# etri/bwa-mem-scale

Hardware: AMD Instinct MI355X
Metric: Mreads/sec through the GPU hot path (seed -> chain -> extend -> dedup, reads and index resident), 150bp SE vs a synthetic genome of GRCh38 size, at 1 MI355X; % HBM roofline in roofline.frac (higher is better)
Workload: dtype int64 intervals / int16 DP (two columns per register; int32 for queries beyond 191 bases or scores beyond 2^14)

## Files before the change

bwa-mem-scale_amd/csrc/api_extend.hip:

```cpp
#include <cstddef>

#include "stage_state.h"

using namespace bwams;

extern "C" {
static int ext_args(bwams_batch *b, StageState *s, const bwams_mem_opt_t *opt, ExtArgs *A) {
    const int64_t n1 = s->ch.nseq + 1;
    A->chains = s->ch.chains.p; A->n_chains = s->ch.n_chains; A->seeds = s->ch.seeds.p; A->n_seeds = s->ch.n_seeds;
    A->chain_off = s->ch.chain_off.as<int64_t>(); A->seed_off = s->ch.chain_off.as<int64_t>() + n1; A->enc = b->d_enc.p; A->cum = b->d_cum.p;
    A->nseq = s->ch.nseq; A->ref = b->idx->fmi.ref;
    int rc = dev_bns(b->idx, &A->bns);
    if (rc) return rc;
    A->opt = *opt; A->regs = s->ext.regs.p; A->srt = s->ext.srt.p; A->rmax = s->ext.rmax.as<int64_t>(); A->cnt = s->ext.cnt.as<int32_t>();
    A->ctr = b->d_ctr.p; A->state = s->ext.state.p; A->kreg = s->ext.kreg.p; A->cur = s->ext.cur.p; A->lim = s->ext.lim.p; A->sel_heavy = s->heavy.p;
    A->n_sel_heavy = &b->d_ctr.p->sel_heavy; A->sel_ticket = b->d_ctr.p->ext_sel_ticket; A->req_list = s->ext.req_list.p; A->rtask = nullptr;
    return BWAMS_OK;
}

static hipError_t ext_round_clear(bwams_batch *b) {
    DevCounters *c = b->d_ctr.p;
    return hipMemsetAsync(&c->ext_n_req, 0, (size_t)((char *)(c->ext_n_retry + 2) - (char *)&c->ext_n_req), b->stream);
}
static int ext_round_fetch(bwams_batch *b, int64_t *n_req, int64_t *n_rest, int64_t *n_l, int64_t *n_r) {
    DevCounters *h = b->h_ctr.p;
    BWAMS_HIP(hipMemcpyAsync(&h->ext_n_req, &b->d_ctr.p->ext_n_req, 3 * sizeof(unsigned long long), hipMemcpyDeviceToHost, b->stream));
    BWAMS_HIP(hipStreamSynchronize(b->stream));
    *n_req = (int64_t)h->ext_n_req; *n_rest = (int64_t)h->ext_n_rest;
    *n_l = (int64_t)(h->ext_n_tasks & 0xffffffffull); *n_r = (int64_t)(h->ext_n_tasks >> 32);
    return BWAMS_OK;
}

static int ext_plan(bwams_batch *b, StageState *s, const bwams_mem_opt_t *opt, int extend_all, ExtArgs *A) {
    const int64_t N1 = s->ch.n_seeds + 1, n1 = s->ch.nseq + 1;
    BWAMS_HIP(s->ext.regs.ensure_n((size_t)N1)); BWAMS_HIP(s->ext.srt.ensure_n((size_t)N1));
    BWAMS_HIP(s->ext.rmax.ensure((size_t)(s->ch.n_chains + 1) * 16)); BWAMS_HIP(s->ext.cnt.ensure((size_t)N1 * 6 * 4));
    BWAMS_HIP(s->ext.state.ensure_n((size_t)N1)); BWAMS_HIP(s->ext.kreg.ensure((size_t)N1 * 32)); BWAMS_HIP(s->ext.cur.ensure_n((size_t)n1));
    BWAMS_HIP(s->ext.lim.ensure_n((size_t)n1)); BWAMS_HIP(s->heavy.ensure_n((size_t)n1));
    BWAMS_HIP(s->ext.req_list.ensure_n((size_t)N1)); BWAMS_HIP(s->ext.rtask.ensure_n((size_t)N1));
    int rc = ext_args(b, s, opt, A);
    if (rc) return rc;
    BWAMS_HIP(hipMemsetAsync(&b->d_ctr.p->sel_heavy, 0, sizeof(unsigned long long), b->stream));
    BWAMS_HIP(ext_round_clear(b));
    launch_ext_heavy_list(*A, b->stream);
    BWAMS_HIP(hipMemsetAsync(s->ext.cur.p, 0, (size_t)n1 * 4, b->stream));
    BWAMS_HIP(hipMemsetAsync(s->ext.lim.p, 0, (size_t)n1 * 4, b->stream));
    launch_ext_plan(*A, extend_all, b->stream);
    return BWAMS_OK;
}

static int ext_build_flat(bwams_batch *b, StageState *s, const ExtArgs &A, const int32_t *list, int64_t n, int64_t tot[6]) {
    hipStream_t st = b->stream;
    const int64_t n1 = n + 1;
    BWAMS_HIP(s->ext.ewide.ensure((size_t)n1 * 6 * 8)); BWAMS_HIP(s->ext.eoffs.ensure((size_t)n1 * 6 * 8));
    launch_ext_widen(A, list, n, s->ext.ewide.as<int64_t>(), st);
    int rc = scan_rows(b, s->ext.ewide.as<int64_t>(), s->ext.eoffs.as<int64_t>(), 6, n1);
    if (rc) return rc;
    for (int r = 0; r < 6; ++r) BWAMS_HIP(hipMemcpyAsync(&tot[r], s->ext.eoffs.as<int64_t>() + r * n1 + n, 8, hipMemcpyDeviceToHost, st));
    BWAMS_HIP(hipStreamSynchronize(st));
    for (int r : {1, 2, 4, 5})
        if (tot[r] >= ((int64_t)1 << 31)) {
            set_last_error("extension task buffers exceed the 31-bit offsets of SeqPair; use smaller chunks");
            return BWAMS_ERR_CAPACITY;
        }
    s->ext.n_left = tot[0]; s->ext.lqer_b = tot[1]; s->ext.lref_b = tot[2];
    s->ext.n_right = tot[3]; s->ext.rqer_b = tot[4]; s->ext.rref_b = tot[5];
    BWAMS_HIP(s->ext.lpairs.ensure_n((size_t)(tot[0] + 1))); BWAMS_HIP(s->ext.rpairs.ensure_n((size_t)(tot[3] + 1)));
    const int64_t mx = tot[0] > tot[3] ? tot[0] : tot[3];
    BWAMS_HIP(s->ext.retry.ensure_n((size_t)(mx + 1)));
    s->ext.tasks_inplace = false;
    BWAMS_HIP(s->ext.lqer.ensure_n((size_t)tot[1] + 64)); BWAMS_HIP(s->ext.lref.ensure_n((size_t)tot[2] + 64));
    BWAMS_HIP(s->ext.rqer.ensure_n((size_t)tot[4] + 64)); BWAMS_HIP(s->ext.rref.ensure_n((size_t)tot[5] + 64));
    if (tot[0] + tot[3] > 0)
        launch_ext_build(A, list, n, s->ext.eoffs.as<int64_t>(), s->ext.lpairs.p, s->ext.lref.p, s->ext.lqer.p, s->ext.rpairs.p, s->ext.rref.p,
                         s->ext.rqer.p, nullptr, nullptr, st);
    return BWAMS_OK;
}

static int ext_build_round(bwams_batch *b, StageState *s, const ExtArgs &A, int64_t n_req, int64_t n_l, int64_t n_r, bool inplace) {
    if (!inplace) {
        int64_t tot[6] = {0, 0, 0, 0, 0, 0};
        if (int rc = ext_build_flat(b, s, A, A.req_list, n_req, tot)) return rc;
        if (tot[0] != n_l || tot[3] != n_r) {
            set_last_error("bwams_extend_run: the request list and its task counters disagree");
            return BWAMS_ERR_DEVICE;
        }
        return BWAMS_OK;
    }
    s->ext.n_left = n_l; s->ext.n_right = n_r;
    s->ext.lqer_b = s->ext.lref_b = s->ext.rqer_b = s->ext.rref_b = 0;
    BWAMS_HIP(s->ext.lpairs.ensure_n((size_t)(n_l + 1))); BWAMS_HIP(s->ext.rpairs.ensure_n((size_t)(n_r + 1)));
    const int64_t mx = n_l > n_r ? n_l : n_r;
    BWAMS_HIP(s->ext.retry.ensure_n((size_t)(mx + 1)));
    s->ext.tasks_inplace = true;
    BWAMS_HIP(s->ext.lsrc.ensure((size_t)(n_l + 1) * 16)); BWAMS_HIP(s->ext.rsrc.ensure((size_t)(n_r + 1) * 16));
    if (n_l + n_r > 0) launch_ext_build(A, A.req_list, n_req, nullptr, s->ext.lpairs.p, nullptr, nullptr, s->ext.rpairs.p,
                         nullptr, nullptr, s->ext.lsrc.as<int64_t>(), s->ext.rsrc.as<int64_t>(), b->stream);
    return BWAMS_OK;
}

int bwams_extend_build(bwams_batch_t *b, const bwams_mem_opt_t *opt, int64_t *n_left, int64_t *n_right) {
    if (!b || !b->stages || !b->stages->ch.done) {
        set_last_error("bwams_extend_build: run bwams_chain_run (or bwams_chain_upload) first");
        return BWAMS_ERR_ARG;
    }
    if (!b->idx->fmi.ref) {
        set_last_error("bwams_extend_build: the index was opened without its .0123 reference");
        return BWAMS_ERR_ARG;
    }
    int rc = check_opt(opt, "bwams_extend_build");
    if (rc) return rc;
    BWAMS_HIP(hipSetDevice(b->idx->device));
    StageState *s = b->stages;
    outdated(s, From::built);
    hipStream_t st = b->stream;
    ExtArgs A;
    BWAMS_HIP(hipEventRecord(s->ev[2], st));
    if ((rc = ext_plan(b, s, opt, 1, &A))) return rc;
    int64_t tot[6];
    if ((rc = ext_build_flat(b, s, A, nullptr, s->ch.n_seeds, tot))) return rc;
    BWAMS_HIP(hipEventRecord(s->ev[3], st));
    BWAMS_HIP(hipGetLastError());
    s->ext.built = true;
    s->opt = *opt;
    if (n_left) *n_left = tot[0];
    if (n_right) *n_right = tot[3];
    return BWAMS_OK;
}

static int run_side(bwams_batch *b, StageState *s, const ExtArgs &A, int right, int64_t *n_retry_out) {
    hipStream_t st = b->stream;
    bwams_seqpair_t *pairs = right ? s->ext.rpairs.p : s->ext.lpairs.p;
    const bool ip = s->ext.tasks_inplace;
    const uint8_t *ref = ip ? A.ref : (right ? s->ext.rref.p : s->ext.lref.p);
    const uint8_t *qer = ip ? A.enc : (right ? s->ext.rqer.p : s->ext.lqer.p);
    const int64_t *src = ip ? (right ? s->ext.rsrc.as<int64_t>() : s->ext.lsrc.as<int64_t>()) : nullptr;
    const int dir = ip && !right ? -1 : 1;
    const int64_t n = right ? s->ext.n_right : s->ext.n_left;
    SwParams prm;
    sw_params(A.opt, right ? A.opt.pen_clip3 : A.opt.pen_clip5, &prm);
    const int qmax = b->max_read_len > 1 ? b->max_read_len : 1;
    if (n == 0) return BWAMS_OK;
    unsigned long long *d_nretry = &b->d_ctr.p->ext_n_retry[right], *h_nretry = &b->h_ctr.p->ext_n_retry[right];
    bwams_seqpair_t *rp = A.rtask ? s->ext.rpairs.p : nullptr;
    if (bsw_list_bytes(n) > b->sw.d_bsw_list.cap) BWAMS_HIP(hipStreamSynchronize(st));
    BWAMS_HIP(b->sw.d_bsw_list.ensure(bsw_list_bytes(n), bsw_list_bytes(n + n / 4 + 1024)));
    if (int lrc = launch_bsw(pairs, n, ref, qer, A.opt.w, prm, qmax, b->d_ctr.p, b->cu_count, st, b->sw.d_bsw_list.p, s->aux, s->fork, s->join, src, dir)) {
        set_last_error(lrc == -2 ? "banded SW: a query longer than ~18000 bases does not fit the LDS kernel" : "banded SW: stream fork/join failed");
        return lrc == -2 ? BWAMS_ERR_UNSUPPORTED : BWAMS_ERR_DEVICE;
    }
    launch_ext_post(A, right, pairs, n, A.opt.w, 0, s->ext.retry.p, d_nretry, rp, st);
    BWAMS_HIP(hipMemcpyAsync(h_nretry, d_nretry, sizeof(unsigned long long), hipMemcpyDeviceToHost, st));
    BWAMS_HIP(hipStreamSynchronize(st));
    const unsigned long long nr = *h_nretry;
    if (nr) {
        if (launch_bsw(s->ext.retry.p, (int64_t)nr, ref, qer, A.opt.w << 1, prm, qmax, b->d_ctr.p, b->cu_count, st, b->sw.d_bsw_list.p, s->aux, s->fork, s->join, src, dir)) return BWAMS_ERR_DEVICE;
        launch_ext_post(A, right, s->ext.retry.p, (int64_t)nr, A.opt.w << 1, 1, nullptr, d_nretry, rp, st);
    }
    *n_retry_out += (int64_t)nr;
    return BWAMS_OK;
}

int bwams_extend_run(bwams_batch_t *b, const bwams_mem_opt_t *opt, int64_t *n_regs) {
    if (!b || !b->stages || !b->stages->ch.done) {
        set_last_error("bwams_extend_run: run bwams_chain_run (or bwams_chain_upload) first");
        return BWAMS_ERR_ARG;
    }
    if (!b->idx->fmi.ref) {
        set_last_error("bwams_extend_run: the index was opened without its .0123 reference");
        return BWAMS_ERR_ARG;
    }
    int rc = check_opt(opt, "bwams_extend_run");
    if (rc) return rc;
    int kMaxRounds = 6;
    if (knobs().ext_max_rounds > 0) kMaxRounds = knobs().ext_max_rounds;
    const bool adaptive_off = knobs().ext_all_rounds != 0;
    const bool inplace_on = knobs().ext_inplace != 0;
    StageState *s = b->stages;
    BWAMS_HIP(hipSetDevice(b->idx->device));
    hipStream_t st = b->stream;
    outdated(s, From::built);
    ExtArgs A;
    BWAMS_HIP(hipEventRecord(s->ev[10], st));
    BWAMS_HIP(hipMemsetAsync(&b->d_ctr.p->bsw_cells, 0, sizeof(unsigned long long), st));
    BWAMS_HIP(hipEventRecord(s->ev[2], st));
    if ((rc = ext_plan(b, s, opt, opt->extend_all != 0, &A))) return rc;
    A.rtask = s->ext.rtask.p;
    int64_t tot_left = 0, tot_right = 0;
    s->ext.n_retry_left = s->ext.n_retry_right = 0;
    int64_t n_req = 0, n_rest = 0, n_l = 0, n_r = 0;
    if ((rc = ext_round_fetch(b, &n_req, &n_rest, &n_l, &n_r))) return rc;
    int round = 0;
    for (;; ++round) {
        if ((rc = ext_build_round(b, s, A, n_req, n_l, n_r, inplace_on))) return rc;
        if (round == 0) { BWAMS_HIP(hipEventRecord(s->ev[3], st)); BWAMS_HIP(hipEventRecord(s->ev[4], st)); }
        tot_left += n_l; tot_right += n_r;
        if ((rc = run_side(b, s, A, 0, &s->ext.n_retry_left))) return rc;
        if (round == 0) { BWAMS_HIP(hipEventRecord(s->ev[5], st)); BWAMS_HIP(hipEventRecord(s->ev[6], st)); }
        if ((rc = run_side(b, s, A, 1, &s->ext.n_retry_right))) return rc;
        if (round == 0) { BWAMS_HIP(hipEventRecord(s->ev[7], st)); BWAMS_HIP(hipEventRecord(s->ev[8], st)); }
        BWAMS_HIP(ext_round_clear(b));
        const bool verbose_sel = knobs().verbose != 0;
        if (verbose_sel) BWAMS_HIP(hipMemsetAsync(b->d_ctr.p->dbg, 0, sizeof b->d_ctr.p->dbg, st));
        if (s->ch.n_seeds && launch_ext_select(A, b->cu_count, st, s->aux, s->fork, s->join)) {
            set_last_error("bwams_extend_run: stream fork/join failed");
            return BWAMS_ERR_DEVICE;
        }
        if (verbose_sel) {
            unsigned long long d[16];
            BWAMS_HIP(hipMemcpyAsync(d, b->d_ctr.p->dbg, sizeof d, hipMemcpyDeviceToHost, st));
            BWAMS_HIP(hipStreamSynchronize(st));
            if (d[0])
                fprintf(stderr, "[bwams_extend_run] selection walk, round %d: %llu reads, Mticks total %.2f fetch %.2f scan %.2f keep-anyway %.2f; %llu slots, %llu chunks, "
                                "%llu keep-anyway calls; longest read: %.3f Mticks (fetch %.3f scan %.3f keep %.3f), %llu slots %llu chunks %llu calls, %llu regions\n",
                        round, d[0], d[1] / 1e6, d[2] / 1e6, d[3] / 1e6, d[4] / 1e6, d[5], d[6], d[7], d[8] / 1e6, d[9] / 1e6, d[10] / 1e6, d[11] / 1e6, d[12], d[13], d[14], d[15]);
        }
        if (round == 0) BWAMS_HIP(hipEventRecord(s->ev[9], st));
        if ((rc = ext_round_fetch(b, &n_req, &n_rest, &n_l, &n_r))) return rc;
        if (n_req == 0) break;
        const bool few_left = !adaptive_off && (n_req + n_rest) * 32 < tot_left + tot_right;
        if (round + 1 >= kMaxRounds || few_left) {
            launch_ext_request_rest(A, st);
            if ((rc = ext_round_fetch(b, &n_req, &n_rest, &n_l, &n_r))) return rc;
        }
    }
    BWAMS_HIP(hipEventRecord(s->ev[11], st));
    BWAMS_HIP(hipGetLastError());
    s->ext.n_rounds = round + 1;
    s->ext.n_left = tot_left; s->ext.n_right = tot_right;
    s->ext.done = true;
    s->opt = *opt;
    if (n_regs) *n_regs = s->ch.n_seeds;
    return BWAMS_OK;
}

int bwams_extend_fetch(bwams_batch_t *b, bwams_alnreg_t *regs, int64_t reg_cap, int64_t *reg_off, int32_t *seed_aln) {
    if (!b || !b->stages || !(b->stages->ext.done || b->stages->ext.built)) {
        set_last_error("bwams_extend_fetch: no regions on the device");
        return BWAMS_ERR_ARG;
    }
    StageState *s = b->stages;
    if (s->ch.n_seeds > reg_cap) return BWAMS_ERR_CAPACITY;
    BWAMS_HIP(hipSetDevice(b->idx->device));
    hipStream_t st = b->stream;
    if (s->ch.n_seeds) BWAMS_HIP(hipMemcpyAsync(regs, s->ext.regs.p, (size_t)s->ch.n_seeds * sizeof(bwams_alnreg_t), hipMemcpyDeviceToHost, st));
    if (reg_off) BWAMS_HIP(hipMemcpyAsync(reg_off, s->ch.chain_off.as<int64_t>() + (s->ch.nseq + 1), (size_t)(s->ch.nseq + 1) * 8, hipMemcpyDeviceToHost, st));
    if (seed_aln && s->ch.n_seeds)
        BWAMS_HIP(hipMemcpy2DAsync(seed_aln, 4, reinterpret_cast<const char *>(s->ch.seeds.p) + offsetof(bwams_chain_seed_t, aln),
                                   sizeof(bwams_chain_seed_t), 4, (size_t)s->ch.n_seeds, hipMemcpyDeviceToHost, st));
    BWAMS_HIP(hipStreamSynchronize(st));
    return BWAMS_OK;
}

int bwams_extend_tasks_fetch(bwams_batch_t *b, int32_t side, bwams_seqpair_t *pairs, int64_t pair_cap, uint8_t *ref,
                             int64_t ref_cap, uint8_t *qer, int64_t qer_cap, int64_t *n_pairs, int64_t *ref_bytes,
                             int64_t *qer_bytes) {
    if (!b || !b->stages || !(b->stages->ext.built || b->stages->ext.done) || (side != 0 && side != 1)) {
        set_last_error("bwams_extend_tasks_fetch: no task lists on the device");
        return BWAMS_ERR_ARG;
    }
    if (b->stages->ext.tasks_inplace) {
        set_last_error("bwams_extend_tasks_fetch: bwams_extend_run extends in place and builds no flat task buffers; bwams_extend_build does");
        return BWAMS_ERR_ARG;
    }
    StageState *s = b->stages;
    const int64_t n = side ? s->ext.n_right : s->ext.n_left, rb = side ? s->ext.rref_b : s->ext.lref_b, qb = side ? s->ext.rqer_b : s->ext.lqer_b;
    if (n_pairs) *n_pairs = n;
    if (ref_bytes) *ref_bytes = rb;
    if (qer_bytes) *qer_bytes = qb;
    if (n > pair_cap || rb > ref_cap || qb > qer_cap) return BWAMS_ERR_CAPACITY;
    BWAMS_HIP(hipSetDevice(b->idx->device));
    hipStream_t st = b->stream;
    if (n) BWAMS_HIP(hipMemcpyAsync(pairs, side ? s->ext.rpairs.p : s->ext.lpairs.p, (size_t)n * sizeof(bwams_seqpair_t), hipMemcpyDeviceToHost, st));
    if (rb) BWAMS_HIP(hipMemcpyAsync(ref, side ? s->ext.rref.p : s->ext.lref.p, (size_t)rb, hipMemcpyDeviceToHost, st));
    if (qb) BWAMS_HIP(hipMemcpyAsync(qer, side ? s->ext.rqer.p : s->ext.lqer.p, (size_t)qb, hipMemcpyDeviceToHost, st));
    BWAMS_HIP(hipStreamSynchronize(st));
    return BWAMS_OK;
}
}
```

bwa-mem-scale_amd/csrc/ext_aln.hip:

```cpp
#include "common.h"
#include "chain_kernels.h"
#include "wave_ops.h"

namespace bwams {
namespace {

constexpr int H0_ = -99;
constexpr int kExtKept = 1, kExtPurged = 2, kExtReq = 4, kExtDone = 8;

__device__ __forceinline__ int cal_max_gap(const bwams_mem_opt_t &o, int qlen) {
    const int l_del = (int)((double)(qlen * o.a - o.o_del) / o.e_del + 1.);
    const int l_ins = (int)((double)(qlen * o.a - o.o_ins) / o.e_ins + 1.);
    int l = l_del > l_ins ? l_del : l_ins;
    l = l > 1 ? l : 1;
    return l < (o.w << 1) ? l : (o.w << 1);
}

__device__ __forceinline__ int pos2rid(const DevBns &b, int64_t pos_f) {
    int left = 0, mid = 0, right = b.n_seqs;
    if (pos_f >= b.l_pac) return -1;
    while (left < right) {
        mid = (left + right) >> 1;
        if (pos_f >= b.contigs[mid].offset) {
            if (mid == b.n_seqs - 1) break;
            if (pos_f < b.contigs[mid + 1].offset) break;
            left = mid + 1;
        } else right = mid;
    }
    return mid;
}

__device__ __forceinline__ int seedcov(const bwams_alnreg_t &a, const bwams_chain_t &c, const bwams_chain_seed_t *seeds) {
    int cov = 0;
    for (int i = 0; i < c.n; ++i) {
        const bwams_chain_seed_t *t = &seeds[c.seed_off + i];
        if (t->qbeg >= a.qb && t->qbeg + t->len <= a.qe && t->rbeg >= a.rb && t->rbeg + t->len <= a.re) cov += t->len;
    }
    return cov;
}

__device__ __forceinline__ unsigned long long ext_block_reserve(unsigned n_mine, unsigned nl, unsigned nr, DevCounters *ctr) {
    __shared__ unsigned int l_n[3];
    __shared__ unsigned long long l_base;
    if (threadIdx.x < 3) l_n[threadIdx.x] = 0;
    __syncthreads();
    unsigned off = 0;
    if (n_mine) {
        off = atomicAdd(&l_n[0], n_mine);
        if (nl) atomicAdd(&l_n[1], nl);
        if (nr) atomicAdd(&l_n[2], nr);
    }
    __syncthreads();
    if (threadIdx.x == 0 && l_n[0]) {
        l_base = atomicAdd(&ctr->ext_n_req, (unsigned long long)l_n[0]);
        atomicAdd(&ctr->ext_n_tasks, (unsigned long long)l_n[1] | ((unsigned long long)l_n[2] << 32));
    }
    __syncthreads();
    return l_base + off;
}

__global__ __launch_bounds__(256) void ext_plan_kernel(ExtArgs A, int extend_all) {
    const int64_t j = (int64_t)blockIdx.x * blockDim.x + threadIdx.x;
    bwams_chain_t c;
    c.n = 0;
    if (j < A.n_chains) c = A.chains[j];
    const bool live = j < A.n_chains && c.n > 0;
    const int r = live ? c.seqid : 0;
    const int l_query = live ? (int)(A.cum[r + 1] - A.cum[r]) : 0;
    const int64_t l_pac = A.bns.l_pac;
    bwams_chain_seed_t *cs = A.seeds + (live ? c.seed_off : 0);
    uint32_t *srt = A.srt + (live ? c.seed_off : 0);
    int64_t r0 = l_pac << 1, r1 = 0;
    unsigned my_req = 0, my_nl = 0, my_nr = 0;
    if (live) {
        for (int i = 0; i < c.n; ++i) {
            const int64_t rb = cs[i].rbeg;
            const int qb = cs[i].qbeg, ln = cs[i].len;
            const int64_t b = rb - (qb + cal_max_gap(A.opt, qb));
            const int64_t e = rb + ln + ((l_query - qb - ln) + cal_max_gap(A.opt, l_query - qb - ln));
            r0 = r0 < b ? r0 : b;
            r1 = r1 > e ? r1 : e;
        }
        r0 = r0 > 0 ? r0 : 0;
        r1 = r1 < (l_pac << 1) ? r1 : (l_pac << 1);
        const int64_t rbeg0 = cs[0].rbeg;
        if (r0 < l_pac && l_pac < r1) {
            if (rbeg0 < l_pac) r1 = l_pac;
            else r0 = l_pac;
        }
        {
            const bool is_rev = rbeg0 >= l_pac;
            const int rid = pos2rid(A.bns, is_rev ? (l_pac << 1) - 1 - rbeg0 : rbeg0);
            int64_t far_beg = A.bns.contigs[rid].offset, far_end = far_beg + A.bns.contigs[rid].len;
            if (is_rev) { const int64_t t0 = far_beg; far_beg = (l_pac << 1) - far_end; far_end = (l_pac << 1) - t0; }
            r0 = r0 > far_beg ? r0 : far_beg;
            r1 = r1 < far_end ? r1 : far_end;
        }
        A.rmax[2 * j] = r0; A.rmax[2 * j + 1] = r1;

        for (int i = 0; i < c.n; ++i) {
            const int sc = cs[i].score;
            int p = i;
            while (p > 0 && cs[srt[p - 1]].score > sc) { srt[p] = srt[p - 1]; --p; }
            srt[p] = (uint32_t)i;
        }
        for (int k = c.n - 1; k >= (extend_all ? 0 : c.n - 1); --k) {
            const bwams_chain_seed_t *s = &cs[srt[k]];
            const unsigned nl = s->qbeg != 0, nr = s->qbeg + s->len != l_query;
            my_req += nl | nr; my_nl += nl; my_nr += nr;
        }
    }
    unsigned long long at = ext_block_reserve(my_req, my_nl, my_nr, A.ctr);
    if (!live) return;

    const int64_t reg0 = A.seed_off[r];
    const int64_t N = A.n_seeds;
    for (int k = c.n - 1; k >= 0; --k) {
        const int64_t p = c.seed_off + (c.n - 1 - k);
        bwams_chain_seed_t *s = &cs[srt[k]];
        s->aln = (int32_t)(p - reg0);
        bwams_alnreg_t a;
        a.rb = a.re = H0_; a.qb = a.qe = H0_;
        a.rid = c.rid; a.pad0_ = 0;
        a.chain = j;
        a.score = a.truesc = -1;
        a.sub = a.alt_sc = a.csub = a.sub_n = 0;
        a.w = A.opt.w; a.seedcov = 0; a.secondary = a.secondary_all = 0;
        a.seedlen0 = s->len; a.n_comp_is_alt = 0;
        a.frac_rep = c.frac_rep; a.pad1_ = 0; a.hash = 0; a.flg = 0; a.pad2_ = 0;
        int nl = 0, lq = 0, lr = 0, nr = 0, rq = 0, rr = 0;
        if (s->qbeg) {
            nl = 1; lq = s->qbeg; lr = (int)(s->rbeg - r0);
            a.qb = s->qbeg; a.rb = s->rbeg;
        } else {
            a.score = a.truesc = s->len * A.opt.a; a.qb = 0; a.rb = s->rbeg;
        }
        if (s->qbeg + s->len != l_query) {
            const int64_t qe = s->qbeg + s->len;
            const int64_t re = s->rbeg + s->len - r0;
            nr = 1; rq = (int)(l_query - qe); rr = (int)(r1 - r0 - re);
            a.qe = (int32_t)qe; a.re = r0 + re;
        } else {
            a.qe = l_query; a.re = s->rbeg + s->len;
            a.seedcov = seedcov(a, c, A.seeds);
        }
        A.regs[p] = a;
        A.cnt[0 * N + p] = nl; A.cnt[1 * N + p] = lq; A.cnt[2 * N + p] = lr;
        A.cnt[3 * N + p] = nr; A.cnt[4 * N + p] = rq; A.cnt[5 * N + p] = rr;
        int st = 0;
        if (!nl && !nr) st = kExtDone;
        else if (extend_all || k == c.n - 1) { st = kExtReq; A.req_list[at++] = (int32_t)p; }
        A.state[p] = st;
    }
}

__global__ void ext_widen_kernel(const int32_t *cnt, const int32_t *state, const int32_t *list, int64_t n_seeds, int64_t n, int64_t *wide) {
    const int64_t g = (int64_t)blockIdx.x * blockDim.x + threadIdx.x;
    if (g >= 6 * (n + 1)) return;
    const int64_t row = g / (n + 1), i = g - row * (n + 1);
    int64_t v = 0;
    if (i < n) {
        const int64_t p = list ? list[i] : i;
        if (list || (state[p] & kExtReq)) v = cnt[row * n_seeds + p];
    }
    wide[g] = v;
}

__device__ __forceinline__ int64_t shfl64(int64_t v, int src) {
    return ((int64_t)__shfl((int)(v >> 32), src) << 32) | (uint32_t)__shfl((int)v, src);
}
constexpr int kBuildBlock = 1024;
__global__ __launch_bounds__(kBuildBlock) void ext_build_kernel(ExtArgs A, const int32_t *__restrict__ list, int64_t n, const int64_t *__restrict__ offs,
                                                               bwams_seqpair_t *left, uint8_t *lref, uint8_t *lqer, bwams_seqpair_t *right,
                                                               uint8_t *rref, uint8_t *rqer, int64_t *lsrc, int64_t *rsrc) {
    __shared__ unsigned int l_cnt[2];
    __shared__ unsigned long long l_base[2];
    const int lane = threadIdx.x & 63;
    const int64_t N = A.n_seeds, n1 = n + 1;
    const int64_t i = (int64_t)blockIdx.x * blockDim.x + threadIdx.x;
    const int64_t p = i < n ? (list ? (int64_t)list[i] : i) : 0;
    const int st = i < n ? A.state[p] : 0;
    const bool req = (st & kExtReq) != 0;
    const int nl = req ? A.cnt[0 * N + p] : 0, nr = req ? A.cnt[3 * N + p] : 0;
    int64_t ti_l = 0, ti_r = 0;
    if (offs) {
        if (nl) ti_l = offs[0 * n1 + i];
        if (nr) ti_r = offs[3 * n1 + i];
    } else {
        if (threadIdx.x < 2) l_cnt[threadIdx.x] = 0;
        __syncthreads();
        unsigned int off_l = 0, off_r = 0;
        const unsigned long long ml = __ballot(nl != 0), mr = __ballot(nr != 0);
        if (ml) {
            const int leader = __ffsll((long long)ml) - 1;
            unsigned int wbase = 0;
            if (lane == leader) wbase = atomicAdd(&l_cnt[0], (unsigned int)__popcll(ml));
            off_l = (unsigned int)__shfl((int)wbase, leader) + (unsigned int)__popcll(ml & ((1ull << lane) - 1ull));
        }
        if (mr) {
            const int leader = __ffsll((long long)mr) - 1;
            unsigned int wbase = 0;
            if (lane == leader) wbase = atomicAdd(&l_cnt[1], (unsigned int)__popcll(mr));
            off_r = (unsigned int)__shfl((int)wbase, leader) + (unsigned int)__popcll(mr & ((1ull << lane) - 1ull));
        }
        __syncthreads();
        if (threadIdx.x < 2 && l_cnt[threadIdx.x]) l_base[threadIdx.x] = atomicAdd(&A.ctr->ext_head[threadIdx.x], (unsigned long long)l_cnt[threadIdx.x]);
        __syncthreads();
        if (nl) ti_l = (int64_t)l_base[0] + off_l;
        if (nr) ti_r = (int64_t)l_base[1] + off_r;
    }
    int64_t l_qsrc = 0, l_rsrc = 0, l_qo = 0, l_ro = 0, r_qsrc = 0, r_rsrc = 0, r_qo = 0, r_ro = 0;
    int l_ql = 0, l_rl = 0, r_ql = 0, r_rl = 0;
    if (req) {
        A.state[p] = (st & ~kExtReq) | kExtDone;
        const int64_t j = A.regs[p].chain;
        const bwams_chain_t c = A.chains[j];
        const int k = c.n - 1 - (int)(p - c.seed_off);
        const bwams_chain_seed_t sd = A.seeds[c.seed_off + A.srt[c.seed_off + k]];
        const int r = c.seqid;
        const int64_t qoff = A.cum[r];
        const int l_query = (int)(A.cum[r + 1] - qoff);
        const int64_t r0 = A.rmax[2 * j];
        if (A.rtask) A.rtask[p] = nr ? (int32_t)ti_r : -1;
        if (nl) {
            if (offs) { l_qo = offs[1 * n1 + i]; l_ro = offs[2 * n1 + i]; }
            l_ql = sd.qbeg; l_rl = (int)(sd.rbeg - r0);
            l_qsrc = qoff + sd.qbeg - 1; l_rsrc = sd.rbeg - 1;
            bwams_seqpair_t sp;
            sp.idr = (int32_t)l_ro; sp.idq = (int32_t)l_qo; sp.id = (int32_t)ti_l;
            sp.len1 = l_rl; sp.len2 = l_ql; sp.h0 = sd.len * A.opt.a; sp.seqid = r; sp.regid = sd.aln;
            sp.score = sp.tle = sp.gtle = sp.qle = sp.gscore = sp.max_off = 0;
            left[ti_l] = sp;
            if (lsrc) { lsrc[2 * ti_l] = l_qsrc; lsrc[2 * ti_l + 1] = l_rsrc; }
        }
        if (nr) {
            if (offs) { r_qo = offs[4 * n1 + i]; r_ro = offs[5 * n1 + i]; }
            const int qe = sd.qbeg + sd.len;
            r_ql = l_query - qe; r_rl = A.cnt[5 * N + p];
            r_qsrc = qoff + qe; r_rsrc = sd.rbeg + sd.len;
            bwams_seqpair_t sp;
            sp.idr = (int32_t)r_ro; sp.idq = (int32_t)r_qo; sp.id = (int32_t)ti_r;
            sp.len1 = r_rl; sp.len2 = r_ql; sp.h0 = (A.rtask && !nl) ? sd.len * A.opt.a : H0_; sp.seqid = r; sp.regid = sd.aln;
            sp.score = sp.tle = sp.gtle = sp.qle = sp.gscore = sp.max_off = 0;
            right[ti_r] = sp;
            if (rsrc) { rsrc[2 * ti_r] = r_qsrc; rsrc[2 * ti_r + 1] = r_rsrc; }
        }
    }
    unsigned long long m = lsrc ? 0ull : __ballot(req);
    while (m) {
        const int src = __ffsll((long long)m) - 1;
        m &= m - 1;
        const int ql = __shfl(l_ql, src), rl = __shfl(l_rl, src), qr = __shfl(r_ql, src), rr = __shfl(r_rl, src);
        if (ql | rl) {
            const int64_t qs = shfl64(l_qsrc, src), rs = shfl64(l_rsrc, src), qo = shfl64(l_qo, src), ro = shfl64(l_ro, src);
            for (int t = lane; t < ql; t += 64) lqer[qo + t] = A.enc[qs - t];
            for (int t = lane; t < rl; t += 64) lref[ro + t] = A.ref[rs - t];
        }
        if (qr | rr) {
            const int64_t qs = shfl64(r_qsrc, src), rs = shfl64(r_rsrc, src), qo = shfl64(r_qo, src), ro = shfl64(r_ro, src);
            for (int t = lane; t < qr; t += 64) rqer[qo + t] = A.enc[qs + t];
            for (int t = lane; t < rr; t += 64) rref[ro + t] = A.ref[rs + t];
        }
    }
}

__global__ __launch_bounds__(256) void ext_post_kernel(ExtArgs A, int right, const bwams_seqpair_t *__restrict__ pairs, int64_t n, int w, int last_try,
                                bwams_seqpair_t *__restrict__ retry, unsigned long long *n_retry, bwams_seqpair_t *__restrict__ rpairs) {
    const int64_t l = (int64_t)blockIdx.x * blockDim.x + threadIdx.x;
    if (l >= n) return;
    struct { int32_t seqid, regid, h0, score, tle, gtle, qle, gscore, max_off; } sp;
    sp.seqid = pairs[l].seqid; sp.regid = pairs[l].regid; sp.h0 = pairs[l].h0; sp.score = pairs[l].score; sp.tle = pairs[l].tle;
    sp.gtle = pairs[l].gtle; sp.qle = pairs[l].qle; sp.gscore = pairs[l].gscore; sp.max_off = pairs[l].max_off;
    const int64_t slot = A.seed_off[sp.seqid] + sp.regid;
    bwams_alnreg_t *ap = &A.regs[slot];
    bwams_alnreg_t a = *ap;
    const int prev = a.score;
    a.score = sp.score;
    if (a.score == prev || sp.max_off < (w >> 1) + (w >> 2) || last_try) {
        if (!right) {
            if (sp.gscore <= 0 || sp.gscore <= a.score - A.opt.pen_clip5) {
                a.qb -= sp.qle; a.rb -= sp.tle;
                a.truesc = a.score;
            } else {
                a.qb = 0; a.rb -= sp.gtle;
                a.truesc = sp.gscore;
            }
            if (rpairs) { const int32_t rt = A.rtask[slot]; if (rt >= 0) rpairs[rt].h0 = a.score; }
        } else {
            if (sp.gscore <= 0 || sp.gscore <= a.score - A.opt.pen_clip3) {
                a.qe += sp.qle; a.re += sp.tle;
                a.truesc += a.score - sp.h0;
            } else {
                a.qe = (int32_t)(A.cum[sp.seqid + 1] - A.cum[sp.seqid]); a.re += sp.gtle;
                a.truesc += sp.gscore - sp.h0;
            }
        }
        a.w = a.w > w ? a.w : w;
        if (a.rb != H0_ && a.qb != H0_ && a.qe != H0_ && a.re != H0_) a.seedcov = seedcov(a, A.chains[a.chain], A.seeds);
        *ap = a;
    } else {
        ap->score = a.score;
        retry[atomicAdd(n_retry, 1ull)] = pairs[l];
    }
}

constexpr int kLightRegs = 32;

__device__ __forceinline__ int purge_class(const bwams_mem_opt_t &opt, const bwams_chain_seed_t &s, int l_query, int64_t prb,
                                           int64_t pre, int pqb, int pqe, int pseedlen0, int pw) {
    if (pqb == -1 && pqe == -1) return 0;
    if (s.rbeg < prb || s.rbeg + s.len > pre || s.qbeg < pqb || s.qbeg + s.len > pqe) return 1;
    if ((double)(s.len - pseedlen0) > .1 * (double)l_query) return 1;
    int qd = s.qbeg - pqb;
    int64_t rd = s.rbeg - prb;
    int max_gap = cal_max_gap(opt, (int)(qd < rd ? qd : rd));
    int w = max_gap < pw ? max_gap : pw;
    if (qd - rd < w && rd - qd < w) return 2;
    qd = pqe - (s.qbeg + s.len); rd = pre - (s.rbeg + s.len);
    max_gap = cal_max_gap(opt, (int)(qd < rd ? qd : rd));
    w = max_gap < pw ? max_gap : pw;
    if (qd - rd < w && rd - qd < w) return 2;
    return 1;
}

__device__ __forceinline__ bool purge_keep_anyway(const bwams_chain_seed_t &s, const bwams_chain_seed_t *cs, const uint32_t *srt2,
                                                  int k, int n) {
    int v;
    for (v = k + 1; v < n; ++v) {
        const uint32_t sv = __hip_atomic_load(&srt2[v], __ATOMIC_RELAXED, __HIP_MEMORY_SCOPE_AGENT);
        if (sv == 0xffffffffu) continue;
        const bwams_chain_seed_t t = cs[sv];
        if ((double)t.len < (double)s.len * .95) continue;
        if (s.qbeg <= t.qbeg && s.qbeg + s.len - t.qbeg >= (s.len >> 2) && t.qbeg - s.qbeg != t.rbeg - s.rbeg) break;
        if (t.qbeg <= s.qbeg && t.qbeg + t.len - s.qbeg >= (s.len >> 2) && s.qbeg - t.qbeg != s.rbeg - t.rbeg) break;
    }
    return v != n;
}

struct KReg { int64_t rb, re; int32_t qb, qe, seedlen0, w; };

__device__ __forceinline__ void select_seed_of_slot(const ExtArgs &A, int64_t p, bwams_chain_t &c, int &k, bwams_chain_seed_t &s) {
    c = A.chains[A.regs[p].chain];
    k = c.n - 1 - (int)(p - c.seed_off);
    const uint32_t sk = __hip_atomic_load(&A.srt[c.seed_off + k], __ATOMIC_RELAXED, __HIP_MEMORY_SCOPE_AGENT);
    s = A.seeds[c.seed_off + sk];
}

__global__ __launch_bounds__(64) void ext_select_kernel(ExtArgs A) {
    const int64_t r = (int64_t)blockIdx.x * blockDim.x + threadIdx.x;
    bool req = false;
    int rest = 0;
    int64_t req_p = 0;
    if (r < A.nseq) {
        const int64_t reg0 = A.seed_off[r];
        const int av_n = (int)(A.seed_off[r + 1] - reg0);
        int t = A.cur[r];
        if (av_n <= kLightRegs && t < av_n) {
            const int l_query = (int)(A.cum[r + 1] - A.cum[r]);
            KReg *kreg = reinterpret_cast<KReg *>(A.kreg) + reg0;
            int lim = A.lim[r];
            for (; t < av_n; ++t) {
                const int64_t p = reg0 + t;
                bwams_chain_t c;
                bwams_chain_seed_t s;
                int k;
                select_seed_of_slot(A, p, c, k, s);
                bool brk = false;
                for (int i = 0; i < lim && !brk; ++i) {
                    const KReg q = kreg[i];
                    brk = purge_class(A.opt, s, l_query, q.rb, q.re, q.qb, q.qe, q.seedlen0, q.w) == 2;
                }
                const int st = A.state[p];
                if (brk && !purge_keep_anyway(s, A.seeds + c.seed_off, A.srt + c.seed_off, k, c.n)) {
                    A.regs[p].qb = -1; A.regs[p].qe = -1;
                    A.srt[c.seed_off + k] = 0xffffffffu;
                    A.state[p] = st | kExtPurged;
                    continue;
                }
                if (!(st & kExtDone)) { A.state[p] = st | kExtReq; req = true; req_p = p; rest = av_n - t - 1; break; }
                const bwams_alnreg_t *a = &A.regs[p];
                KReg q;
                q.rb = a->rb; q.re = a->re; q.qb = a->qb; q.qe = a->qe; q.seedlen0 = a->seedlen0; q.w = a->w;
                kreg[lim++] = q;
                A.state[p] = st | kExtKept;
            }
            A.cur[r] = t;
            A.lim[r] = lim;
        }
    }
    const unsigned long long m = __ballot(req);
    if (m) {
        const int lane = threadIdx.x & 63, leader = __ffsll((long long)m) - 1;
        int nl = req ? A.cnt[0 * A.n_seeds + req_p] : 0, nr = req ? A.cnt[3 * A.n_seeds + req_p] : 0;
        for (int o = 32; o > 0; o >>= 1) { rest += __shfl_xor(rest, o); nl += __shfl_xor(nl, o); nr += __shfl_xor(nr, o); }
        unsigned long long base = 0;
        if (lane == leader) {
            base = atomicAdd(&A.ctr->ext_n_req, (unsigned long long)__popcll(m));
            atomicAdd(&A.ctr->ext_n_tasks, (unsigned long long)(unsigned)nl | ((unsigned long long)(unsigned)nr << 32));
            if (rest) atomicAdd(&A.ctr->ext_n_rest, (unsigned long long)rest);
        }
        base = (unsigned long long)shfl64((int64_t)base, leader);
        if (req) A.req_list[base + (unsigned long long)__popcll(m & ((1ull << lane) - 1ull))] = (int32_t)req_p;
    }
}

__global__ void ext_heavy_list_kernel(ExtArgs A) {
    const int64_t r = (int64_t)blockIdx.x * blockDim.x + threadIdx.x;
    if (r >= A.nseq) return;
    if (A.seed_off[r + 1] - A.seed_off[r] > kLightRegs) A.sel_heavy[atomicAdd(A.n_sel_heavy, 1ull)] = (int32_t)r;
}

__device__ __forceinline__ bool purge_keep_anyway_w(const bwams_chain_seed_t &s, const bwams_chain_seed_t *cs, const uint32_t *srt2, int k, int n,
                                                    int lane) {
    bool found = false;
    for (int v0 = k + 1; v0 < n && !found; v0 += 64) {
        const int v = v0 + lane;
        bool hit = false;
        if (v < n) {
            const uint32_t sv = __hip_atomic_load(&srt2[v], __ATOMIC_RELAXED, __HIP_MEMORY_SCOPE_AGENT);
            if (sv != 0xffffffffu) {
                const bwams_chain_seed_t t = cs[sv];
                if (!((double)t.len < (double)s.len * .95)) {
                    hit = (s.qbeg <= t.qbeg && s.qbeg + s.len - t.qbeg >= (s.len >> 2) && t.qbeg - s.qbeg != t.rbeg - s.rbeg) ||
                          (t.qbeg <= s.qbeg && t.qbeg + t.len - s.qbeg >= (s.len >> 2) && s.qbeg - t.qbeg != s.rbeg - t.rbeg);
                }
            }
        }
        found = __any(hit);
    }
    return found;
}

constexpr int kSelCap[3] = {256, 640, 1280};
constexpr int kSelSteps = 4;
__global__ __launch_bounds__(64) void ext_select_wave_kernel(ExtArgs A, int lo, int cap, unsigned long long *ticket) {
    extern __shared__ __align__(16) unsigned char l_sel_raw[];
    KReg *lk = reinterpret_cast<KReg *>(l_sel_raw);
    const int lane = threadIdx.x & 63;
    const int64_t n_heavy = (int64_t)*A.n_sel_heavy;
    for (;;) {
        const int64_t ti = (int64_t)wave_ticket(ticket, 1ull);
        if (ti >= n_heavy) break;
        const int64_t r = A.sel_heavy[ti];
        const int64_t reg0 = A.seed_off[r];
        const int av_n = (int)(A.seed_off[r + 1] - reg0);
        if (av_n <= lo || (av_n > cap && cap != kSelCap[2])) continue;
        int t = A.cur[r];
        if (t >= av_n) continue;
        const int l_query = (int)(A.cum[r + 1] - A.cum[r]);
        KReg *kreg = reinterpret_cast<KReg *>(A.kreg) + reg0;
        int lim = A.lim[r];
        const bool in_lds = av_n <= cap;
        __syncthreads();
        if (in_lds)
            for (int i = lane; i < lim; i += 64) lk[i] = kreg[i];
        __syncthreads();
        bool stop = false;
#ifdef BWAMS_SELDBG
        const unsigned long long T0 = __builtin_amdgcn_s_memtime();
        unsigned long long t_scan = 0, n_slots = 0, n_chunks = 0;
#endif
        while (t < av_n && !stop) {
            const int nb = av_n - t < 64 ? av_n - t : 64;
            int64_t my_off = 0, my_rbeg = 0;
            int my_n = 0, my_k = 0, my_st = 0, my_qbeg = 0, my_len = 0;
            if (lane < nb) {
                const int64_t p = reg0 + t + lane;
                bwams_chain_t c;
                bwams_chain_seed_t sd;
                select_seed_of_slot(A, p, c, my_k, sd);
                my_off = c.seed_off; my_n = c.n; my_rbeg = sd.rbeg; my_qbeg = sd.qbeg; my_len = sd.len;
                my_st = A.state[p];
            }
            int j = 0;
            for (; j < nb; ++j) {
                const int64_t p = reg0 + t + j;
                const int64_t c_off = ((int64_t)__shfl((int)(my_off >> 32), j) << 32) | (uint32_t)__shfl((int)my_off, j);
                bwams_chain_seed_t s;
                s.rbeg = ((int64_t)__shfl((int)(my_rbeg >> 32), j) << 32) | (uint32_t)__shfl((int)my_rbeg, j);
                s.qbeg = __shfl(my_qbeg, j); s.len = __shfl(my_len, j);
                const int c_n = __shfl(my_n, j), k = __shfl(my_k, j), st = __shfl(my_st, j);
                bool brk = false;
#ifdef BWAMS_SELDBG
                const unsigned long long Tb = __builtin_amdgcn_s_memtime();
                ++n_slots;
#endif
                for (int base = 0; base < lim && !brk; base += 64 * kSelSteps) {
                    KReg q[kSelSteps];
                    bool go[kSelSteps];
#pragma unroll
                    for (int u = 0; u < kSelSteps; ++u) {
                        const int i = base + u * 64 + lane;
                        const int ii = i < lim ? i : lim - 1;
                        q[u] = in_lds ? lk[ii] : kreg[ii];
                        go[u] = (i < lim) & !((q[u].qb == -1) & (q[u].qe == -1)) &
                                !((s.rbeg < q[u].rb) | (s.rbeg + s.len > q[u].re) | (s.qbeg < q[u].qb) | (s.qbeg + s.len > q[u].qe));
                    }
                    bool hit = false;
#pragma unroll
                    for (int u = 0; u < kSelSteps; ++u)
                        if (go[u]) hit |= purge_class(A.opt, s, l_query, q[u].rb, q[u].re, q[u].qb, q[u].qe, q[u].seedlen0, q[u].w) == 2;
                    brk = __ballot(hit) != 0;
#ifdef BWAMS_SELDBG
                    n_chunks += kSelSteps;
#endif
                }
#ifdef BWAMS_SELDBG
                t_scan += __builtin_amdgcn_s_memtime() - Tb;
#endif
                if (brk && !purge_keep_anyway_w(s, A.seeds + c_off, A.srt + c_off, k, c_n, lane)) {
                    if (lane == 0) {
                        __hip_atomic_store(reinterpret_cast<unsigned long long *>(&A.regs[p].qb), 0xffffffffffffffffull,
                                           __ATOMIC_RELAXED, __HIP_MEMORY_SCOPE_AGENT);
                        __hip_atomic_store(&A.srt[c_off + k], 0xffffffffu, __ATOMIC_RELAXED, __HIP_MEMORY_SCOPE_AGENT);
                        A.state[p] = st | kExtPurged;
                    }
                    continue;
                }
                if (!(st & kExtDone)) {
                    if (lane == 0) {
                        A.state[p] = st | kExtReq;
                        A.req_list[atomicAdd(&A.ctr->ext_n_req, 1ull)] = (int32_t)p;
                        atomicAdd(&A.ctr->ext_n_tasks, (unsigned long long)(unsigned)A.cnt[0 * A.n_seeds + p] |
                                                           ((unsigned long long)(unsigned)A.cnt[3 * A.n_seeds + p] << 32));
                        if (av_n - (t + j) - 1 > 0) atomicAdd(&A.ctr->ext_n_rest, (unsigned long long)(av_n - (t + j) - 1));
                    }
                    stop = true;
                    break;
                }
                if (lane == 0) {
                    const bwams_alnreg_t *a = &A.regs[p];
                    KReg q;
                    q.rb = a->rb; q.re = a->re; q.qb = a->qb; q.qe = a->qe; q.seedlen0 = a->seedlen0; q.w = a->w;
                    kreg[lim] = q;
                    if (in_lds) lk[lim] = q;
                    A.state[p] = st | kExtKept;
                }
                ++lim;
                __syncthreads();
            }
            t += j;
        }
        if (lane == 0) { A.cur[r] = t; A.lim[r] = lim; }
#ifdef BWAMS_SELDBG
        if (lane == 0) {
            const unsigned long long tot = __builtin_amdgcn_s_memtime() - T0;
            unsigned long long *d = A.ctr->dbg;
            atomicAdd(&d[0], 1ull); atomicAdd(&d[1], tot); atomicAdd(&d[3], t_scan); atomicAdd(&d[5], n_slots); atomicAdd(&d[6], n_chunks);
            if (atomicMax(&d[8], tot) < tot) { d[10] = t_scan; d[12] = n_slots; d[13] = n_chunks; d[15] = (unsigned long long)av_n; }
        }
#endif
    }
}

__global__ __launch_bounds__(256) void ext_request_rest_kernel(ExtArgs A) {
    const int64_t p = (int64_t)blockIdx.x * blockDim.x + threadIdx.x;
    const int st = p < A.n_seeds ? A.state[p] : kExtDone;
    const bool want = !(st & (kExtKept | kExtPurged | kExtDone | kExtReq));
    const unsigned nl = want ? (unsigned)A.cnt[0 * A.n_seeds + p] : 0u, nr = want ? (unsigned)A.cnt[3 * A.n_seeds + p] : 0u;
    const unsigned long long at = ext_block_reserve(want ? 1u : 0u, nl, nr, A.ctr);
    if (want) { A.state[p] = st | kExtReq; A.req_list[at] = (int32_t)p; }
}

}

void launch_ext_plan(const ExtArgs &A, int extend_all, hipStream_t st) {
    if (A.n_chains > 0) ext_plan_kernel<<<(unsigned)((A.n_chains + 255) / 256), 256, 0, st>>>(A, extend_all);
}
void launch_ext_widen(const ExtArgs &A, const int32_t *list, int64_t n, int64_t *wide, hipStream_t st) {
    const int64_t g = 6 * (n + 1);
    ext_widen_kernel<<<(unsigned)((g + 255) / 256), 256, 0, st>>>(A.cnt, A.state, list, A.n_seeds, n, wide);
}

void launch_ext_build(const ExtArgs &A, const int32_t *list, int64_t n, const int64_t *offs, bwams_seqpair_t *left, uint8_t *lref, uint8_t *lqer,
                      bwams_seqpair_t *right, uint8_t *rref, uint8_t *rqer, int64_t *lsrc, int64_t *rsrc, hipStream_t st) {
    if (n <= 0) return;
    ext_build_kernel<<<(unsigned)((n + kBuildBlock - 1) / kBuildBlock), kBuildBlock, 0, st>>>(A, list, n, offs, left, lref, lqer, right, rref, rqer,
                                                                                              lsrc, rsrc);
}

void launch_ext_post(const ExtArgs &A, int right, const bwams_seqpair_t *pairs, int64_t n, int w, int last_try,
                     bwams_seqpair_t *retry, unsigned long long *n_retry, bwams_seqpair_t *rpairs, hipStream_t st) {
    if (n <= 0) return;
    ext_post_kernel<<<(unsigned)((n + 255) / 256), 256, 0, st>>>(A, right, pairs, n, w, last_try, retry, n_retry, right ? nullptr : rpairs);
}

void launch_ext_heavy_list(const ExtArgs &A, hipStream_t st) {
    if (A.nseq <= 0) return;
    ext_heavy_list_kernel<<<(unsigned)((A.nseq + 255) / 256), 256, 0, st>>>(A);
}
int launch_ext_select(const ExtArgs &A, int cu_count, hipStream_t st, hipStream_t *aux, hipEvent_t fork, hipEvent_t *join) {
    if (A.nseq <= 0) return 0;
    if (hipEventRecord(fork, st) != hipSuccess || hipStreamWaitEvent(aux[0], fork, 0) != hipSuccess) return -1;
    ext_select_wave_kernel<<<(unsigned)(cu_count * 3), 64, kSelCap[2] * sizeof(KReg), aux[0]>>>(A, kSelCap[1], kSelCap[2], A.sel_ticket + 2);
    ext_select_kernel<<<(unsigned)((A.nseq + 63) / 64), 64, 0, st>>>(A);
    ext_select_wave_kernel<<<(unsigned)(cu_count * 7), 64, kSelCap[1] * sizeof(KReg), st>>>(A, kSelCap[0], kSelCap[1], A.sel_ticket + 1);
    ext_select_wave_kernel<<<(unsigned)(cu_count * 16), 64, kSelCap[0] * sizeof(KReg), st>>>(A, kLightRegs, kSelCap[0], A.sel_ticket);
    if (hipEventRecord(join[0], aux[0]) != hipSuccess || hipStreamWaitEvent(st, join[0], 0) != hipSuccess) return -1;
    return 0;
}
void launch_ext_request_rest(const ExtArgs &A, hipStream_t st) {
    if (A.n_seeds <= 0) return;
    ext_request_rest_kernel<<<(unsigned)((A.n_seeds + 255) / 256), 256, 0, st>>>(A);
}

}
```

Measured before the change: 9.927.

## Restructure extend selection walk into per-lane bulk scan plus ordered incremental check

The selection kernel used to walk candidate slots one at a time, and for each slot the whole wave scanned all kept regions. Now each lane owns one slot of a 64-slot batch and scans the already-kept regions itself with an unrolled loop. An ordered pass then resolves keep-anyway rescue, request, or keep in slot order, and each newly kept region is tested incrementally only against the later lanes. The per-slot barrier and shuffles are replaced by one barrier per batch and readlane broadcasts. This trades the wave-parallel inner scan for per-lane serial scans, which may run slowly when the kept list is long and lanes diverge.

```diff
diff --git a/bwa-mem-scale_amd/csrc/api_extend.hip b/bwa-mem-scale_amd/csrc/api_extend.hip
--- a/bwa-mem-scale_amd/csrc/api_extend.hip
+++ b/bwa-mem-scale_amd/csrc/api_extend.hip
@@ -211,9 +211,11 @@
             BWAMS_HIP(hipMemcpyAsync(d, b->d_ctr.p->dbg, sizeof d, hipMemcpyDeviceToHost, st));
             BWAMS_HIP(hipStreamSynchronize(st));
             if (d[0])
-                fprintf(stderr, "[bwams_extend_run] selection walk, round %d: %llu reads, Mticks total %.2f fetch %.2f scan %.2f keep-anyway %.2f; %llu slots, %llu chunks, "
-                                "%llu keep-anyway calls; longest read: %.3f Mticks (fetch %.3f scan %.3f keep %.3f), %llu slots %llu chunks %llu calls, %llu regions\n",
-                        round, d[0], d[1] / 1e6, d[2] / 1e6, d[3] / 1e6, d[4] / 1e6, d[5], d[6], d[7], d[8] / 1e6, d[9] / 1e6, d[10] / 1e6, d[11] / 1e6, d[12], d[13], d[14], d[15]);
+                fprintf(stderr, "[bwams_extend_run] selection walk, round %d: %llu reads, Mticks total %.2f fetch %.2f bulk scan %.2f ordered part %.2f (of it keep-anyway %.2f); "
+                                "%llu slots, %llu keep-anyway calls; longest read: %.3f Mticks (fetch %.3f bulk %.3f ordered %.3f, of it keep-anyway %.3f), %llu slots "
+                                "%llu calls, %llu kept regions\n",
+                        round, d[0], d[1] / 1e6, d[2] / 1e6, d[3] / 1e6, d[4] / 1e6, d[5] / 1e6, d[6], d[7], d[8] / 1e6, d[9] / 1e6, d[10] / 1e6, d[11] / 1e6,
+                        d[12] / 1e6, d[13], d[14], d[15]);
         }
         if (round == 0) BWAMS_HIP(hipEventRecord(s->ev[9], st));
         if ((rc = ext_round_fetch(b, &n_req, &n_rest, &n_l, &n_r))) return rc;
diff --git a/bwa-mem-scale_amd/csrc/ext_aln.hip b/bwa-mem-scale_amd/csrc/ext_aln.hip
--- a/bwa-mem-scale_amd/csrc/ext_aln.hip
+++ b/bwa-mem-scale_amd/csrc/ext_aln.hip
@@ -432,7 +432,37 @@
 }
 
 constexpr int kSelCap[3] = {256, 640, 1280};
-constexpr int kSelSteps = 4;
+constexpr int kSelUnroll = 6;
+
+__device__ __forceinline__ int64_t readlane64(int64_t v, int j) {
+    return ((int64_t)__builtin_amdgcn_readlane((int)(v >> 32), j) << 32) | (uint32_t)__builtin_amdgcn_readlane((int)v, j);
+}
+
+__device__ __forceinline__ bool sel_contains(const KReg &q, const bwams_chain_seed_t &s) {
+    return !((q.qb == -1) & (q.qe == -1)) & !((s.rbeg < q.rb) | (s.rbeg + s.len > q.re) | (s.qbeg < q.qb) | (s.qbeg + s.len > q.qe));
+}
+
+__device__ __forceinline__ bool sel_bulk_scan(const bwams_mem_opt_t &opt, const KReg *src, int n, const bwams_chain_seed_t &s, int l_query, bool own,
+                                              bool hit) {
+    for (int base = 0; base < n; base += kSelUnroll) {
+        KReg q[kSelUnroll];
+        bool go[kSelUnroll], any = false;
+#pragma unroll
+        for (int u = 0; u < kSelUnroll; ++u) {
+            const int i = base + u;
+            q[u] = src[i < n ? i : n - 1];
+            go[u] = own & sel_contains(q[u], s);
+            any |= go[u];
+        }
+        if (any & !hit) {
+#pragma unroll
+            for (int u = 0; u < kSelUnroll; ++u)
+                if (go[u] && !hit) hit = purge_class(opt, s, l_query, q[u].rb, q[u].re, q[u].qb, q[u].qe, q[u].seedlen0, q[u].w) == 2;
+        }
+    }
+    return hit;
+}
+
 __global__ __launch_bounds__(64) void ext_select_wave_kernel(ExtArgs A, int lo, int cap, unsigned long long *ticket) {
     extern __shared__ __align__(16) unsigned char l_sel_raw[];
     KReg *lk = reinterpret_cast<KReg *>(l_sel_raw);
@@ -458,64 +488,64 @@
         bool stop = false;
 #ifdef BWAMS_SELDBG
         const unsigned long long T0 = __builtin_amdgcn_s_memtime();
-        unsigned long long t_scan = 0, n_slots = 0, n_chunks = 0;
+        unsigned long long t_fetch = 0, t_bulk = 0, t_ord = 0, t_keep = 0, n_slots = 0, n_calls = 0;
 #endif
         while (t < av_n && !stop) {
             const int nb = av_n - t < 64 ? av_n - t : 64;
-            int64_t my_off = 0, my_rbeg = 0;
-            int my_n = 0, my_k = 0, my_st = 0, my_qbeg = 0, my_len = 0;
-            if (lane < nb) {
+            const bool own = lane < nb;
+#ifdef BWAMS_SELDBG
+            const unsigned long long Ta = __builtin_amdgcn_s_memtime();
+#endif
+            bwams_chain_seed_t s;
+            s.rbeg = 0; s.qbeg = 0; s.len = 0;
+            KReg mine;
+            mine.rb = mine.re = 0; mine.qb = mine.qe = mine.seedlen0 = mine.w = 0;
+            int64_t my_off = 0;
+            int my_n = 0, my_k = 0, my_st = 0;
+            if (own) {
                 const int64_t p = reg0 + t + lane;
                 bwams_chain_t c;
                 bwams_chain_seed_t sd;
                 select_seed_of_slot(A, p, c, my_k, sd);
-                my_off = c.seed_off; my_n = c.n; my_rbeg = sd.rbeg; my_qbeg = sd.qbeg; my_len = sd.len;
+                my_off = c.seed_off; my_n = c.n; s.rbeg = sd.rbeg; s.qbeg = sd.qbeg; s.len = sd.len;
                 my_st = A.state[p];
+                const bwams_alnreg_t *a = &A.regs[p];
+                mine.rb = a->rb; mine.re = a->re; mine.qb = a->qb; mine.qe = a->qe; mine.seedlen0 = a->seedlen0; mine.w = a->w;
             }
+#ifdef BWAMS_SELDBG
+            asm volatile("s_waitcnt vmcnt(0)" ::: "memory");
+            const unsigned long long Tb = __builtin_amdgcn_s_memtime();
+#endif
+            bool hit = in_lds ? sel_bulk_scan(A.opt, lk, lim, s, l_query, own, false) : sel_bulk_scan(A.opt, kreg, lim, s, l_query, own, false);
+#ifdef BWAMS_SELDBG
+            const unsigned long long Tc = __builtin_amdgcn_s_memtime();
+#endif
             int j = 0;
             for (; j < nb; ++j) {
                 const int64_t p = reg0 + t + j;
-                const int64_t c_off = ((int64_t)__shfl((int)(my_off >> 32), j) << 32) | (uint32_t)__shfl((int)my_off, j);
-                bwams_chain_seed_t s;
-                s.rbeg = ((int64_t)__shfl((int)(my_rbeg >> 32), j) << 32) | (uint32_t)__shfl((int)my_rbeg, j);
-                s.qbeg = __shfl(my_qbeg, j); s.len = __shfl(my_len, j);
-                const int c_n = __shfl(my_n, j), k = __shfl(my_k, j), st = __shfl(my_st, j);
-                bool brk = false;
-#ifdef BWAMS_SELDBG
-                const unsigned long long Tb = __builtin_amdgcn_s_memtime();
-                ++n_slots;
-#endif
-                for (int base = 0; base < lim && !brk; base += 64 * kSelSteps) {
-                    KReg q[kSelSteps];
-                    bool go[kSelSteps];
-#pragma unroll
-                    for (int u = 0; u < kSelSteps; ++u) {
-                        const int i = base + u * 64 + lane;
-                        const int ii = i < lim ? i : lim - 1;
-                        q[u] = in_lds ? lk[ii] : kreg[ii];
-                        go[u] = (i < lim) & !((q[u].qb == -1) & (q[u].qe == -1)) &
-                                !((s.rbeg < q[u].rb) | (s.rbeg + s.len > q[u].re) | (s.qbeg < q[u].qb) | (s.qbeg + s.len > q[u].qe));
+                const int st = __builtin_amdgcn_readlane(my_st, j);
+                if ((__ballot(hit) >> j) & 1ull) {
+                    bwams_chain_seed_t sj;
+                    sj.rbeg = readlane64(s.rbeg, j); sj.qbeg = __builtin_amdgcn_readlane(s.qbeg, j); sj.len = __builtin_amdgcn_readlane(s.len, j);
+                    const int64_t c_off = readlane64(my_off, j);
+                    const int c_n = __builtin_amdgcn_readlane(my_n, j), k = __builtin_amdgcn_readlane(my_k, j);
+#ifdef BWAMS_SELDBG
+                    const unsigned long long Tk = __builtin_amdgcn_s_memtime();
+                    ++n_calls;
+#endif
+                    const bool rescued = purge_keep_anyway_w(sj, A.seeds + c_off, A.srt + c_off, k, c_n, lane);
+#ifdef BWAMS_SELDBG
+                    t_keep += __builtin_amdgcn_s_memtime() - Tk;
+#endif
+                    if (!rescued) {
+                        if (lane == 0) {
+                            __hip_atomic_store(reinterpret_cast<unsigned long long *>(&A.regs[p].qb), 0xffffffffffffffffull,
+                                               __ATOMIC_RELAXED, __HIP_MEMORY_SCOPE_AGENT);
+                            __hip_atomic_store(&A.srt[c_off + k], 0xffffffffu, __ATOMIC_RELAXED, __HIP_MEMORY_SCOPE_AGENT);
+                            A.state[p] = st | kExtPurged;
+                        }
+                        continue;
                     }
-                    bool hit = false;
-#pragma unroll
-                    for (int u = 0; u < kSelSteps; ++u)
-                        if (go[u]) hit |= purge_class(A.opt, s, l_query, q[u].rb, q[u].re, q[u].qb, q[u].qe, q[u].seedlen0, q[u].w) == 2;
-                    brk = __ballot(hit) != 0;
-#ifdef BWAMS_SELDBG
-                    n_chunks += kSelSteps;
-#endif
-                }
-#ifdef BWAMS_SELDBG
-                t_scan += __builtin_amdgcn_s_memtime() - Tb;
-#endif
-                if (brk && !purge_keep_anyway_w(s, A.seeds + c_off, A.srt + c_off, k, c_n, lane)) {
-                    if (lane == 0) {
-                        __hip_atomic_store(reinterpret_cast<unsigned long long *>(&A.regs[p].qb), 0xffffffffffffffffull,
-                                           __ATOMIC_RELAXED, __HIP_MEMORY_SCOPE_AGENT);
-                        __hip_atomic_store(&A.srt[c_off + k], 0xffffffffu, __ATOMIC_RELAXED, __HIP_MEMORY_SCOPE_AGENT);
-                        A.state[p] = st | kExtPurged;
-                    }
-                    continue;
                 }
                 if (!(st & kExtDone)) {
                     if (lane == 0) {
@@ -528,26 +558,35 @@
                     stop = true;
                     break;
                 }
-                if (lane == 0) {
-                    const bwams_alnreg_t *a = &A.regs[p];
-                    KReg q;
-                    q.rb = a->rb; q.re = a->re; q.qb = a->qb; q.qe = a->qe; q.seedlen0 = a->seedlen0; q.w = a->w;
-                    kreg[lim] = q;
-                    if (in_lds) lk[lim] = q;
+                KReg q;
+                q.rb = readlane64(mine.rb, j); q.re = readlane64(mine.re, j);
+                q.qb = __builtin_amdgcn_readlane(mine.qb, j); q.qe = __builtin_amdgcn_readlane(mine.qe, j);
+                q.seedlen0 = __builtin_amdgcn_readlane(mine.seedlen0, j); q.w = __builtin_amdgcn_readlane(mine.w, j);
+                if (lane == j) {
+                    kreg[lim] = mine;
+                    if (in_lds) lk[lim] = mine;
                     A.state[p] = st | kExtKept;
                 }
+                if (own & (lane > j) & !hit & sel_contains(q, s)) hit = purge_class(A.opt, s, l_query, q.rb, q.re, q.qb, q.qe, q.seedlen0, q.w) == 2;
                 ++lim;
-                __syncthreads();
             }
+#ifdef BWAMS_SELDBG
+            n_slots += (unsigned long long)(j < nb ? j + 1 : j);
+            t_fetch += Tb - Ta; t_bulk += Tc - Tb; t_ord += __builtin_amdgcn_s_memtime() - Tc;
+#endif
             t += j;
+            __syncthreads();
         }
         if (lane == 0) { A.cur[r] = t; A.lim[r] = lim; }
 #ifdef BWAMS_SELDBG
         if (lane == 0) {
             const unsigned long long tot = __builtin_amdgcn_s_memtime() - T0;
             unsigned long long *d = A.ctr->dbg;
-            atomicAdd(&d[0], 1ull); atomicAdd(&d[1], tot); atomicAdd(&d[3], t_scan); atomicAdd(&d[5], n_slots); atomicAdd(&d[6], n_chunks);
-            if (atomicMax(&d[8], tot) < tot) { d[10] = t_scan; d[12] = n_slots; d[13] = n_chunks; d[15] = (unsigned long long)av_n; }
+            atomicAdd(&d[0], 1ull); atomicAdd(&d[1], tot); atomicAdd(&d[2], t_fetch); atomicAdd(&d[3], t_bulk); atomicAdd(&d[4], t_ord);
+            atomicAdd(&d[5], t_keep); atomicAdd(&d[6], n_slots); atomicAdd(&d[7], n_calls);
+            if (atomicMax(&d[8], tot) < tot) {
+                d[9] = t_fetch; d[10] = t_bulk; d[11] = t_ord; d[12] = t_keep; d[13] = n_slots; d[14] = n_calls; d[15] = (unsigned long long)lim;
+            }
         }
 #endif
     }
```

Result: faster. 10.03 (median of 6 runs) (+1.1%).
